# hassony2/homan

Hardware: AMD Instinct MI355X
Metric: optimisation iters/sec (30-frame 256^2 clip) (higher is better)
Workload: dtype f32

## Files before the change

### homan_amd/csrc/raster_api.hip

```cpp
#include "raster_ws.h"

RasterTune& hm_raster_tune()
{
    static thread_local RasterTune t = {0, 0, SWEEP_BLOCKS};
    return t;
}
int& hm_sweep_cap_override()
{
    static int cap = 0;
    return cap;
}
static hipEvent_t g_tev[6];
static int g_timing = 0;
#define HM_TIME_MARK(k, stream) do { if (g_timing) (void)hipEventRecord(g_tev[k], stream); } while (0)

extern "C" {

size_t hm_sil_workspace_bytes(int B, int V, int F, int S)
{
    const size_t is = 2 * (size_t)S;
    size_t n = 256;
    n += al256((size_t)B * 16);
    n += al256((size_t)B * V * 3 * 4);
    n += al256((size_t)B * F * 9 * 4);
    n += al256((size_t)B * F * 8);
    n += al256((size_t)B * is * is * 4);
    n += al256((size_t)B * is * (is / 16) * 2);
    n += al256((size_t)B * S * S * 4);
    n += al256((size_t)B * (S / 8) * (S / 8) * 16);
    n += al256((size_t)B * is * is * 4);
    n += al256((size_t)B * is * (is / 16) * 4);
    n += al256((size_t)B * is * (is / 16) * 4);
    n += al256((size_t)B * F * 24 * 4);
    n += al256((size_t)B * F * 2);
    n += al256((size_t)B * SR_MAX * 8);
    n += al256((size_t)B * (S / 16) * (S / 16));
    n += al256((size_t)B * SR_MAX * F * 4);
    n += al256(4 * (size_t)B * is * (is / 64) * 16);
    n += al256((size_t)B * 2 * is * 16);
    n += al256(4 * (size_t)B * is * is * sizeof(SweepSrc));
    n += al256((size_t)B * F * sizeof(SweepFace));
    n += al256((size_t)B * F * 4) * 2;
    n += al256(sweep_ucap(B, F) * 4);
    n += al256(sweep_slot_cap(B, F) * 24);
    n += al256(ts_units(B, F, S) * 16);
    n += al256(ts_raster_units(B, S) * 4) * 3;
    return n;
}

int hm_tune_raster_lds_pad(int bytes)
{
    const int prev = hm_raster_tune().raster_lds_pad;
    if (bytes >= 0) hm_raster_tune().raster_lds_pad = bytes;
    return prev;
}
int hm_tune_raster_reorder(int enable)
{
    const int prev = hm_raster_tune().raster_reorder;
    if (enable >= 0) hm_raster_tune().raster_reorder = enable ? 1 : 0;
    return prev;
}

int hm_tune_sweep_blocks(int blocks)
{
    const int prev = hm_raster_tune().sweep_blocks;
    if (blocks > 0) hm_raster_tune().sweep_blocks = blocks;
    return prev;
}

int hm_sil_fwd_phase_clips(const float* verts, const int* faces, int faces_bstride, const float* K, int B, int V, int F, int S,
                           float orig_size, float znear, float zfar, const float* keep, const float* ref,
                           const float* keep_sum, float* pooled, float* loss_out, const int* work_order, float* pooled_depth,
                           float* alpha_full, int mask_shared, const float* rigid_rot6d, const float* rigid_trans,
                           const float* rigid_scale, int rigid_abs, int persistent_outputs, void* workspace, int clip_len,
                           int out_stride, float* cam_verts_out, int phases, hipStream_t stream)
{
    HM_CHECK_ARG(phases >= 1 && phases <= 3);
    HM_CHECK_ARG(verts && faces && K && pooled && workspace && HM_CLIP_LEN_OK(B, clip_len));
    if (clip_len == 0) clip_len = B;
// ... 318 lines not shown
```

### homan_amd/csrc/raster_lines.hip

```cpp
#include "raster_ws.h"

__global__ __launch_bounds__(256) void k_bwd_masks(const float* __restrict__ gin, int mode,
                                                   const float* __restrict__ upstream,
                                                   const float* __restrict__ keep_sum, int B, int S,
                                                   const unsigned short* __restrict__ alpha16,
                                                   float* __restrict__ gimg, unsigned short* __restrict__ planes,
                                                   int clip_len)
{
    if (mode == 1 && upstream[0] > 0.0f) return;
    const int w = threadIdx.x >> 6, lane = threadIdx.x & 63;
    const int is = 2 * S, tiles_x = S / HM_TILE, ntiles = tiles_x * tiles_x;
    const int tile = blockIdx.x * 4 + w, b = blockIdx.y;
    if (tile >= ntiles) return;
    const int ty = tile / tiles_x, tx = tile % tiles_x;
    const int rr = lane >> 3, cc = lane & 7;
    const int r = ty * HM_TILE + rr, c = tx * HM_TILE + cc;
    const long po = ((long)b * S + r) * S + c;
    unsigned long long cq[4];
#pragma unroll
    for (int dy = 0; dy < 2; ++dy) {
        const unsigned aw = alpha16[(((long)b * (is / 16) + ty) * (is / 16) + tx) * 16 + 2 * rr + dy];
#pragma unroll
        for (int dx = 0; dx < 2; ++dx) cq[2 * dy + dx] = __ballot((aw >> (2 * cc + dx)) & 1u);
    }
// ... 75 lines not shown
    __shared__ unsigned long long s_base;
    const int tid = threadIdx.x, lane = tid & 63, wv = tid >> 6;
    const int per_clip = nblk / (B / clip_len), clip = blk / per_clip;
    const long cbase = (long)clip * clip_len * F;
    const long bf0 = cbase + ((long)(blk - clip * per_clip) * 256 + tid) * fpt, nbf = cbase + (long)clip_len * F;
    int nk[4], n = 0, hasf = 0;
#pragma unroll
    for (int k = 0; k < 4; ++k) {
        SweepFace rec;
        nk[k] = (k < fpt && bf0 + k < nbf) ? sweep_face_record(bf0 + k, faces9, boxes, owned, F, is, rec) : 0;
        n += nk[k];
        hasf += nk[k] > 0 ? 1 : 0;
    }
    const int inc_i = hm_wave_scan_incl(n), inc_f = hm_wave_scan_incl(hasf);
    if (lane == 63) { s_wsum[wv][0] = inc_i; s_wsum[wv][1] = inc_f; }
    __syncthreads();
    int pre_i = 0, pre_f = 0, tot_i = 0, tot_f = 0;
#pragma unroll
    for (int k = 0; k < 4; ++k) {
        if (k < wv) { pre_i += s_wsum[k][0]; pre_f += s_wsum[k][1]; }
        tot_i += s_wsum[k][0];
        tot_f += s_wsum[k][1];
    }
    if (tid == 0)
        s_base = tot_f ? atomicAdd(sl.cnt, ((unsigned long long)tot_f << 32) | (unsigned)((tot_i + SWEEP_UNIT - 1) & ~(SWEEP_UNIT - 1))) : 0ull;
    __syncthreads();
    const unsigned long long base = s_base;
    int off = (int)(base & 0xffffffffull) + pre_i + inc_i - n;
    int idx = (int)(base >> 32) + pre_f + inc_f - hasf;
#pragma unroll
    for (int k = 0; k < 4; ++k) {
        const long bf = bf0 + k;
        if (k >= fpt || bf >= nbf) break;
        bool zero = nk[k] == 0;
        if (nk[k] > 0) {
            SweepFace rec;
            const int nn = sweep_face_record(bf, faces9, boxes, owned, F, is, rec);
            const int u_lo = off >> SWEEP_USHIFT, u_hi = (off + nn - 1) >> SWEEP_USHIFT;
            const bool over = u_hi >= sl.ucap || u_hi + idx >= sl.slot_cap;
            rec.off = off;
            rec.flags = over ? 1 : 0;
            zero = u_hi > u_lo;
            const uint4* r4 = reinterpret_cast<const uint4*>(&rec);
            uint4* t4 = reinterpret_cast<uint4*>(sl.tab + idx);
#pragma unroll
            for (int q = 0; q < 4; ++q) t4[q] = r4[q];
            sl.offs[idx] = off;
            for (int u = (off + SWEEP_UNIT - 1) >> SWEEP_USHIFT; (u << SWEEP_USHIFT) < off + nn && u < sl.ucap; ++u)
                sl.ufirst[u] = (unsigned)idx;
            off += nn;
            ++idx;
        }
        if (zero) {
            double* o = parts + bf * 6;
#pragma unroll
            for (int q = 0; q < 6; ++q) o[q] = 0.0;
        }
    }
    if (tid == 0) {
        const unsigned int t = atomicAdd(sl.done, 1u);
        if (t == (unsigned)nblk - 1u) {
            sl.total[0] = atomicExch(sl.cnt, 0ull);
            atomicExch(sl.done, 0u);
        }
    }
}


#ifndef LINES_NL
#define LINES_NL 2
#endif
#ifdef LINES_REVERSED
#define LINES_BLK(i, n) ((n) - 1 - (i))
#else
#define LINES_BLK(i, n) (i)
#endif
template <bool W32>
__global__ __launch_bounds__(256) void k_bwd_lines(const unsigned short* __restrict__ planes,
                                                   const float* __restrict__ gimg, const float* __restrict__ dimg,
                                                   int mode, const float* __restrict__ upstream,
                                                   const float* __restrict__ keep_sum,
                                                   const int* __restrict__ idx_map, int B, int S,
                                                   SweepSrc* __restrict__ srcs, uint4* __restrict__ lrec,
                                                   int ncomp, int fpt, const float* __restrict__ faces9,
                                                   const FaceBox* __restrict__ boxes,
                                                   const unsigned char* __restrict__ owned, int F,
// ... 165 lines not shown
```

### homan_amd/csrc/raster_sweep.hip

```cpp
#include "raster_ws.h"
#include "raster_hooks.h"

__device__ __forceinline__ float sample_grad(const float* __restrict__ gimg, int S, int is, int xi, int yi)
{
    return 0.25f * gimg[(long)((is - 1 - yi) >> 1) * S + (xi >> 1)];
}

__device__ __forceinline__ void sweep_term(float diff, int d1, float d1_cross, float k0, float k1, bool use0, bool use1,
                                           float eps, double magic, double& acc0, double& acc1)
{
    const float t = (float)d1 - d1_cross;
    const bool live = diff > 0.0f;
    float dist0 = k0 * t, dist1 = k1 * t;
    dist0 += (0.0f < dist0) ? eps : -eps;
    dist1 += (0.0f < dist1) ? eps : -eps;
    const float g0 = diff / dist0, g1 = diff / dist1;
    acc0 -= hm_quant((live && use0) ? g0 : 0.0f, magic);
    acc1 -= hm_quant((live && use1) ? g1 : 0.0f, magic);
}
__device__ __forceinline__ float sweep_item_scale(float c, float two_over_is, bool pow2, int is)
{
    return pow2 ? (c * 2.0f) * two_over_is : (c * 2.0f) / (float)is;
}

__device__ __forceinline__ void raster_reorder(int* __restrict__ wo_dyn, int* __restrict__ wo_tmp,
                                               const unsigned int* __restrict__ wg_cost, unsigned int* __restrict__ dyn_flag, int n,
                                               unsigned* __restrict__ s_hist)
{
    __shared__ unsigned s_wsum[4];
    __shared__ unsigned s_zero;
    const int tid = threadIdx.x, lane = tid & 63, wv = tid >> 6;
    for (int i = tid; i < 1024; i += 256) s_hist[i] = 0u;
    if (tid == 0) s_zero = 0u;
    __syncthreads();
// ... 125 lines not shown
    q.geo = geo;
    return q;
}

#ifndef SWEEP_COMBINE_MIN
#define SWEEP_COMBINE_MIN 32
#endif
#ifndef SWEEP_COMBINE_PAIRS
#define SWEEP_COMBINE_PAIRS 192
#endif
__device__ __forceinline__ double sweep_row_sum(double v)
{
    v += hm_dpp_f64<0xb1, 0xf>(v);
    v += hm_dpp_f64<0x4e, 0xf>(v);
    v += hm_dpp_f64<0x114, 0xf>(v);
    v += hm_dpp_f64<0x118, 0xf>(v);
    return v;
}
__device__ __forceinline__ void sweep_combine_rows(int& cur, double& acc0, double& acc1, bool flush, int lane)
{
    const unsigned long long nb = __ballot(flush);
    if (__popcll(nb) < SWEEP_COMBINE_MIN) return;
    const int prev = __builtin_amdgcn_update_dpp(cur, cur, 0x111, 0xf, 0xf, false);
    const unsigned long long same = __ballot(prev == cur);
    const int sh = lane & 48;
    const bool uni = ((unsigned)(nb >> sh) & (unsigned)(same >> sh) & 0xffffu) == 0xffffu;
    const double r0 = sweep_row_sum(acc0), r1 = sweep_row_sum(acc1);
    if (uni) {
        if ((lane & 15) == 15) { acc0 = r0; acc1 = r1; }
        else { cur = -1; acc0 = 0.0; acc1 = 0.0; }
    }
}

#ifndef SWEEP_WAVES_EU
#define SWEEP_WAVES_EU 5
#endif
template <bool W32>
__global__ __launch_bounds__(256) __attribute__((amdgpu_waves_per_eu(SWEEP_WAVES_EU, 8))) void k_bwd_sweep(SweepList sl, const int* __restrict__ idx_map,
                                                   const SweepSrc* __restrict__ srcs,
                                                   const uint4* __restrict__ lrec, int B, int F, int S,
                                                   float eps, double magic, double* __restrict__ parts,
                                                   const unsigned short* __restrict__ lsum,
                                                   const unsigned short* __restrict__ alpha16,
                                                   const unsigned int* __restrict__ ts_flag,
                                                   unsigned long long* __restrict__ ts_slots, int nsort,
                                                   int* __restrict__ wo_dyn, int* __restrict__ wo_tmp,
                                                   const unsigned int* __restrict__ wg_cost,
                                                   unsigned int* __restrict__ dyn_flag, int n_wo)
{
    HM_CHAIN_KERNEL();
    typedef typename HmOff<W32>::t OFF;
    const unsigned long long ts_t0 = (unsigned long long)wall_clock64();
    const bool ts_on = hm_ts_enabled(ts_flag) && (threadIdx.x & 63) == 0;
    if (ts_on) hm_ts_store(ts_slots, (long)blockIdx.x * 4 + (threadIdx.x >> 6), 0, ts_t0);
    struct FaceLds { SweepFace f; int pad; };
    struct ItemLds { SweepItem it; int pad; };
    __shared__ FaceLds s_face[4][SWEEP_PASS_FACES];
    __shared__ double s_fg[4][SWEEP_PASS_FACES][6];
    __shared__ int s_start[4][64];
    __shared__ int s_head[4][256];
    __shared__ ItemLds s_item[4][64];
    __shared__ unsigned short s_q[4][SWEEP_UNIT];
    __shared__ int2 s_fam[4][SWEEP_PASS_FACES][12];
    __shared__ int s_fb[4][SWEEP_PASS_FACES][2];
    if (nsort && blockIdx.x == 0) {
        raster_reorder(wo_dyn, wo_tmp, wg_cost, dyn_flag, n_wo, reinterpret_cast<unsigned*>(&s_head[0][0]));
        if (ts_on) hm_ts_store(ts_slots, (long)blockIdx.x * 4 + (threadIdx.x >> 6), 1, (unsigned long long)wall_clock64());
        return;
    }
    const int wid = (int)blockIdx.x - nsort, nwork = (int)gridDim.x - nsort;
    const int lane = threadIdx.x & 63, wv = threadIdx.x >> 6;
    const int is = 2 * S;
    const bool pow2 = (is & (is - 1)) == 0;
    const float inv_is = 1.0f / (float)is;
    const int wpl = is / 64;
    const unsigned long long tot = sl.total[0];
    const int N = (int)(tot & 0xffffffffull), W = (int)(tot >> 32);
    const int U = (N + SWEEP_UNIT - 1) >> SWEEP_USHIFT;
    const int xcd = wid & 7;
    const int xwaves = (nwork >> 3) * 4;
    const int u_end = (int)(((long)U * (xcd + 1)) >> 3);
    int first_ahead = -1;
    for (int u = __builtin_amdgcn_readfirstlane((int)(((long)U * xcd) >> 3) + (wid >> 3) * 4 + wv); u < u_end;
         u += xwaves) {
        const int ubeg = u << SWEEP_USHIFT, uend = ubeg + SWEEP_UNIT;
#ifdef SWEEP_UNIT_PROFILE
        const unsigned long long up_t0 = wall_clock64();
        int up_pass = 0, up_trips = 0, up_q = 0, up_rounds = 0;
#endif
        int first = first_ahead;
        if (first < 0) {
            if (u < sl.ucap) first = (int)sl.ufirst[u];
            else {
                int lo = 0, hi = W - 1;
                while (lo < hi) {
                    const int mid = (lo + hi + 1) >> 1;
                    if (sl.offs[mid] <= ubeg) lo = mid; else hi = mid - 1;
                }
                first = lo;
            }
            first = __builtin_amdgcn_readfirstlane(first);
        }
        const int u_ahead = u + xwaves;
        int ahead_v = -1;
        if (u_ahead < u_end && u_ahead < sl.ucap) ahead_v = (int)sl.ufirst[u_ahead];
        for (int fb = 0;; fb += SWEEP_PASS_FACES) {
            const int o = (lane <= SWEEP_PASS_FACES && first + fb + lane < W) ? sl.offs[first + fb + lane] : 0x7fffffff;
            int row[SWEEP_PASS_FACES / 4];
#pragma unroll
            for (int k = 0; k < SWEEP_PASS_FACES / 4; ++k) {
                const int fi = first + fb + 4 * k + (lane >> 4);
                row[k] = fi < W ? reinterpret_cast<const int*>(sl.tab + fi)[lane & 15] : 0;
            }
            if (fb == 0) first_ahead = __builtin_amdgcn_readfirstlane(ahead_v);
            const int nfp = __popcll(__ballot(lane < SWEEP_PASS_FACES && o < uend));
            if (nfp == 0) break;
#ifdef SWEEP_UNIT_PROFILE
            ++up_pass;
// ... 153 lines not shown
                if (on[ph]) {
                    rf[ph] = *hm_at<W32>(lrec, lid[ph] * wpl + (rfrom[ph] >> 6));
                    rt[ph] = *hm_at<W32>(lrec, lid[ph] * wpl + (rto[ph] >> 6));
                }
            }
#pragma unroll
            for (int ph = 0; ph < 2; ++ph) {
                const unsigned long long wf = rf[ph].x | ((unsigned long long)rf[ph].y << 32);
                const unsigned long long wt = rt[ph].x | ((unsigned long long)rt[ph].y << 32);
                lo[ph] = (int)rf[ph].z + __popcll(wf & ((1ull << (rfrom[ph] & 63)) - 1ull));
                nbp[ph] = on[ph] ? (int)rt[ph].z + __popcll(wt & (~0ull >> (63 - (rto[ph] & 63)))) - lo[ph] : 0;
            }
            const int nb0 = nbp[0], nb1 = nbp[1];
#ifdef SWEEP_STATS
            {
                const unsigned long long c[7] = {__popcll(__ballot(mine)), __popcll(__ballot(geo)), __popcll(__ballot(act0)),
                                                 __popcll(__ballot(act1)), __popcll(__ballot(nb0 > 0)), __popcll(__ballot(nb1 > 0)),
                                                 (unsigned long long)hm_wave_scan_incl(nb0 + nb1)};
                if (lane == 63) { for (int k = 0; k < 7; ++k) atomicAdd(&g_sweep_n[k], c[k]); atomicAdd(&g_sweep_n[7], 1ull); }
            }
#endif
            const int n = nb0 + nb1;
            const int incl = hm_wave_scan_incl(n);
            const int npairs = __builtin_amdgcn_readlane(incl, 63);
            if (npairs > 0) {
                __builtin_amdgcn_wave_barrier();
                s_start[wv][lane] = incl - n;
                SweepItem it;
                it.x = d1_cross;
                it.c0 = sweep_item_scale(c0, inv_is, pow2, is);
                it.c1 = sweep_item_scale(c1, inv_is, pow2, is);
                it.base0 = (int)(lid[0] * is) + lo[0];
                it.base1 = (int)(lid[1] * is) + lo[1];
                it.nb0 = nb0;
                it.fn = fn;
                {
                    const int m0 = var ? 2 - edge : edge, k1 = edge == 2 ? 0 : edge + 1, m1 = var ? 2 - k1 : k1;
                    const int comp = axis ? 0 : 1;
                    it.meta = el | ((2 * m0 + comp) << 4) | ((2 * m1 + comp) << 7) | (use0 ? 1 << 10 : 0) |
                              (use1 ? 1 << 11 : 0) | (nb0 << 12);
                }
                s_item[wv][lane].it = it;
                wave_sync();
                const int* st = s_start[wv];
                int cur = -1;
                double acc0 = 0.0, acc1 = 0.0;
                int carry = 0;
#pragma unroll 1
                for (int base = 0; base < npairs; base += 256) {
                    SWEEP_HOOK_PAIR_ROUND(eps, base);
#ifdef SWEEP_STATS
                    if (lane == 0) atomicAdd(&g_sweep_n[11], 1ull);
#endif
#ifdef SWEEP_UNIT_PROFILE
                    ++up_rounds;
#endif
                    int4* hd = reinterpret_cast<int4*>(s_head[wv]);
                    hd[lane] = make_int4(0, 0, 0, 0);
                    wave_sync();
                    const int ex = incl - n;
                    if (n > 0 && ex >= base && ex < base + 256) s_head[wv][ex - base] = lane + 1;
                    wave_sync();
                    const int4 h = hd[lane];
                    int m[4];
                    m[0] = h.x; m[1] = max(m[0], h.y); m[2] = max(m[1], h.z); m[3] = max(m[2], h.w);
                    int inc = m[3];
                    inc = max(inc, __builtin_amdgcn_update_dpp(0, inc, 0x111, 0xf, 0xf, false));
                    inc = max(inc, __builtin_amdgcn_update_dpp(0, inc, 0x112, 0xf, 0xf, false));
                    inc = max(inc, __builtin_amdgcn_update_dpp(0, inc, 0x114, 0xf, 0xf, false));
                    inc = max(inc, __builtin_amdgcn_update_dpp(0, inc, 0x118, 0xf, 0xf, false));
                    inc = max(inc, __builtin_amdgcn_update_dpp(0, inc, 0x142, 0xa, 0xf, false));
                    inc = max(inc, __builtin_amdgcn_update_dpp(0, inc, 0x143, 0xc, 0xf, false));
                    int before = __builtin_amdgcn_update_dpp(0, inc, 0x138, 0xf, 0xf, false);
                    before = max(before, carry);
                    carry = max(carry, __builtin_amdgcn_readlane(inc, 63));
                    SweepSrc sc[4];
                    int qi[4], qmeta[4];
                    bool ph1[4];
#pragma unroll
                    for (int k = 0; k < 4; ++k) {
                        const int p = min(base + 4 * lane + k, npairs - 1);
                        const int i = max(max(before, m[k]) - 1, 0);
                        const int r = max(p - st[i], 0);
                        const SweepItem& qq = s_item[wv][i].it;
                        qmeta[k] = qq.meta;
                        const int q_nb0 = qmeta[k] >> 12;
                        ph1[k] = r >= q_nb0;
                        qi[k] = i;
                        OFF at = (OFF)qq.base0 + r;
                        if (ph1[k]) at = (OFF)qq.base1 + (r - q_nb0);
                        sc[k] = *hm_at<W32>(srcs, at);
                    }
#if SWEEP_COMBINE_MIN <= 64
                    if (base > 0) {
                        const int key0 = base + 4 * lane < npairs ? (qmeta[0] & 0x3ff) : cur;
                        sweep_combine_rows(cur, acc0, acc1, cur >= 0 && key0 != cur, lane);
                    }
#endif
#pragma unroll
                    for (int k = 0; k < 4; ++k) {
                        {
                            const bool valid = base + 4 * lane + k < npairs;
                            const SweepItem& qq = s_item[wv][qi[k]].it;
                            const int meta = qmeta[k], key = valid ? (meta & 0x3ff) : cur;
                            if (key != cur) {
                                if (cur >= 0) {
#ifdef SWEEP_HOOK_FLUSH
                                    SWEEP_HOOK_FLUSH(eps, s_fg[wv], lane, cur, acc0, acc1);
#else
                                    double* f = s_fg[wv][cur & 15];
                                    unsafeAtomicAdd(f + ((cur >> 4) & 7), acc0);
                                    unsafeAtomicAdd(f + ((cur >> 7) & 7), acc1);
#endif
                                }
                                cur = key;
                                acc0 = 0.0;
                                acc1 = 0.0;
                            }
                            const bool take = valid && (!ph1[k] || sc[k].owner == qq.fn);
                            sweep_term(take ? (ph1[k] ? sc[k].g : -sc[k].g) : 0.0f, sc[k].d1, qq.x, qq.c0, qq.c1,
                                       (meta & (1 << 10)) != 0, (meta & (1 << 11)) != 0, eps, magic, acc0, acc1);
                        }
                    }
                }
#if SWEEP_COMBINE_MIN <= 64
                if (npairs >= SWEEP_COMBINE_PAIRS) sweep_combine_rows(cur, acc0, acc1, cur >= 0, lane);
#endif
                if (cur >= 0) {
                    double* f = s_fg[wv][cur & 15];
                    unsafeAtomicAdd(f + ((cur >> 4) & 7), acc0);
                    unsafeAtomicAdd(f + ((cur >> 7) & 7), acc1);
                }
            }
            wave_sync();
            }
            if (lane < nfp) {
                const SweepFace& ff = s_face[wv][lane].f;
                const int off = ff.off, nit = (int)ff.cum[11];
                const int u_lo = off >> SWEEP_USHIFT, u_hi = (off + nit - 1) >> SWEEP_USHIFT;
                double v[6];
#pragma unroll
                for (int k = 0; k < 6; ++k) v[k] = s_fg[wv][lane][k];
                double* out = parts + (long)ff.bf * 6;
                if (u_lo == u_hi) {
#pragma unroll
                    for (int k = 0; k < 6; ++k) out[k] = v[k];
                } else {
#pragma unroll
                    for (int k = 0; k < 6; ++k) unsafeAtomicAdd(out + k, v[k]);
                }
            }
            if (nfp < SWEEP_PASS_FACES) break;
        }
#ifdef SWEEP_UNIT_PROFILE
        if (lane == 0 && u < 65536) {
            g_unit_prof[u][0] = (int)(wall_clock64() - up_t0); g_unit_prof[u][1] = up_pass;
            g_unit_prof[u][2] = up_trips | (up_q << 8); g_unit_prof[u][3] = up_rounds;
        }
#endif
    }
    if (ts_on) hm_ts_store(ts_slots, (long)blockIdx.x * 4 + (threadIdx.x >> 6), 1, (unsigned long long)wall_clock64());
}

__global__ void k_bwd_gather(const double* __restrict__ parts, const int* __restrict__ adj_off,
                             const int* __restrict__ adj_items, const float* __restrict__ verts,
                             const float* __restrict__ K, int B, int V, int F, float orig_size,
                             float* __restrict__ grad_ndc, float* __restrict__ grad_verts)
{
    const long i = (long)blockIdx.x * blockDim.x + threadIdx.x;
    if (i >= (long)B * V) return;
    const int b = (int)(i / V), v = (int)(i % V);
    double su = 0.0, sv = 0.0;
    const double2* pf = reinterpret_cast<const double2*>(parts + (long)b * F * 6);
    const int a1 = adj_off[v + 1];
    for (int a = adj_off[v]; a < a1; a += 8) {
        int item[8];
#pragma unroll
        for (int k = 0; k < 8; ++k) item[k] = a + k < a1 ? adj_items[a + k] : -1;
        double2 g2[8];
#pragma unroll
        for (int k = 0; k < 8; ++k) g2[k] = item[k] >= 0 ? pf[item[k]] : make_double2(0.0, 0.0);
#pragma unroll
        for (int k = 0; k < 8; ++k) { su += g2[k].x; sv += g2[k].y; }
    }
    const float gu = (float)su, gv = (float)sv;
    if (grad_ndc) { grad_ndc[3 * i] = gu; grad_ndc[3 * i + 1] = gv; grad_ndc[3 * i + 2] = 0.f; }
    const float* k = K + b * 9;
    const float x = verts[3 * i], y = verts[3 * i + 1], z = verts[3 * i + 2];
    const float zz = z + 1e-9f;
    const float du0 = gu * (2.0f / orig_size), dv0 = -gv * (2.0f / orig_size);
    const float dxn = k[0] * du0 + k[3] * dv0;
    const float dyn = k[1] * du0 + k[4] * dv0;
    grad_verts[3 * i] = dxn / zz;
    grad_verts[3 * i + 1] = dyn / zz;
    grad_verts[3 * i + 2] = -(dxn * x + dyn * y) / (zz * zz);
}

void hm_launch_sweep(const SilWs& w, int B, int F, int S, float eps, int sum_log2q, hipStream_t stream)
{
    const RasterTune& tune = hm_raster_tune();
    const int nsort = tune.raster_reorder ? 1 : 0;
    const int blocks = max(8, (min(min(hm_cdiv((long)B * F, 2), tune.sweep_blocks), TS_SWEEP_WGS - 8) & ~7) - 8 * nsort);
    const bool w32 = hm_offsets_fit_32(B, S);
    hipLaunchKernelGGL(w32 ? k_bwd_sweep<true> : k_bwd_sweep<false>, dim3(nsort + blocks), dim3(256), 0, stream, w.sweep,
                       w.idx_map, w.srcs, w.lrec, B, F, S, eps, hm_sum_magic(sum_log2q), w.parts, w.lsum, w.alpha16, w.counter + 24,
                       w.ts + 2 * (ts_raster_units(B, S) + ts_lines_units(B, F, S)), nsort, w.wo_dyn, w.wo_tmp, w.wg_cost,
                       w.counter + 26, (int)ts_raster_units(B, S));
}
void hm_launch_bwd_gather(const SilWs& w, const int* adj_off, const int* adj_items, const float* verts, const float* K, int B,
                          int V, int F, float orig_size, float* grad_ndc, float* grad_verts, hipStream_t stream)
{
    hipLaunchKernelGGL(k_bwd_gather, dim3(hm_cdiv((long)B * V, 256)), dim3(256), 0, stream, w.parts, adj_off, adj_items, verts,
                       K, B, V, F, orig_size, grad_ndc, grad_verts);
}
int hm_sweep_occupancy(int* blocks_per_cu)
{
    return hipOccupancyMaxActiveBlocksPerMultiprocessor(blocks_per_cu, k_bwd_sweep<true>, 256, 0) == hipSuccess ? HM_OK : HM_ERR_LAUNCH;
}
#ifdef SWEEP_UNIT_PROFILE
extern "C" int hm_debug_unit_profile(int* out)
{
    (void)hipDeviceSynchronize();
    (void)hipMemcpyFromSymbol(out, HIP_SYMBOL(g_unit_prof), sizeof(int) * 65536 * 4);
    static int z[65536][4];
    (void)hipMemcpyToSymbol(HIP_SYMBOL(g_unit_prof), z, sizeof(z));
    return HM_OK;
}
#endif
#ifdef SWEEP_STATS
extern "C" int hm_debug_sweep_stats(unsigned long long* out)
{
    unsigned long long z[16] = {0, 0, 0, 0, 0, 0, 0, 0, 0, 0, 0, 0, 0, 0, 0, 0};
    (void)hipDeviceSynchronize();
    (void)hipMemcpyFromSymbol(out, HIP_SYMBOL(g_sweep_n), sizeof(z));
    (void)hipMemcpyToSymbol(HIP_SYMBOL(g_sweep_n), z, sizeof(z));
    return HM_OK;
}
#endif
```

### homan_amd/csrc/raster_ws.h

```cpp
#pragma once
#include "raster_common.h"

#define HM_INTERNAL __attribute__((visibility("hidden")))

#ifndef SWEEP_BLOCKS
#define SWEEP_BLOCKS 1280
#endif
struct RasterTune {
    int raster_lds_pad;
    int raster_reorder;
    int sweep_blocks;
};
HM_INTERNAL RasterTune& hm_raster_tune();
HM_INTERNAL int& hm_sweep_cap_override();
#define TS_SWEEP_WGS 4096
static inline size_t ts_raster_units(int B, int S) { return (size_t)B * (S / 8) * (S / 8) / RASTER_WAVES; }
static inline size_t ts_lines_units(int B, int F, int S) { return (size_t)B * F / 256 + 2 * (size_t)B + 64 + (size_t)B * S / 2 + 8; }
static inline size_t ts_units(int B, int F, int S) { return ts_raster_units(B, S) + ts_lines_units(B, F, S) + 4 * TS_SWEEP_WGS; }
static inline size_t sweep_ucap(int B, int F) { return (size_t)B * F * 4 + 1024; }
static inline size_t sweep_slot_cap(int B, int F) { return sweep_ucap(B, F) + (size_t)B * F; }

static inline size_t al256(size_t x) { return (x + 255) & ~(size_t)255; }

struct SilWs {
    unsigned int* counter; float* frame_rec;
    float* ndc; float* faces9; FaceBox* boxes; int* idx_map; unsigned short* alpha16; float* dimg;
    float* partials; float* gimg; unsigned short* planes; double* parts;
    unsigned char* owned; int* bin_cnt; unsigned int* bin_done; unsigned char* region_state; int* bin_list;
    uint4* lrec; SweepSrc* srcs; unsigned short* lsum;
    SweepList sweep;
    unsigned long long* ts;
    int* wo_dyn; int* wo_tmp; unsigned int* wg_cost;
};
static inline SilWs carve(void* ws, int B, int V, int F, int S)
{
    const size_t is = 2 * (size_t)S;
    char* p = (char*)ws;
    SilWs w;
    w.counter = (unsigned int*)p; p += 256;
    w.frame_rec = (float*)p; p += al256((size_t)B * 16);
    w.ndc = (float*)p; p += al256((size_t)B * V * 3 * 4);
    w.faces9 = (float*)p; p += al256((size_t)B * F * 9 * 4);
    w.boxes = (FaceBox*)p; p += al256((size_t)B * F * 8);
    w.idx_map = (int*)p; p += al256((size_t)B * is * is * 4);
    w.alpha16 = (unsigned short*)p; p += al256((size_t)B * is * (is / 16) * 2);
    w.dimg = (float*)p; p += al256((size_t)B * S * S * 4);
    w.partials = (float*)p; p += al256((size_t)B * (S / 8) * (S / 8) * 16);
    w.gimg = (float*)p; p += al256((size_t)B * is * is * 4);
    w.planes = (unsigned short*)p; p += al256((size_t)B * is * (is / 16) * 4) * 2;
    w.parts = (double*)p; p += al256((size_t)B * F * 24 * 4);
    w.owned = (unsigned char*)p; p += al256((size_t)B * F * 2);
    w.bin_cnt = (int*)p; w.bin_done = (unsigned int*)(p + (size_t)B * SR_MAX * 4); p += al256((size_t)B * SR_MAX * 8);
    w.region_state = (unsigned char*)p; p += al256((size_t)B * (S / 16) * (S / 16));
    w.bin_list = (int*)p; p += al256((size_t)B * SR_MAX * F * 4);
    w.lrec = (uint4*)p; p += al256(4 * (size_t)B * is * (is / 64) * 16);
    w.lsum = (unsigned short*)p; p += al256((size_t)B * 2 * is * 16);
    w.srcs = (SweepSrc*)p; p += al256(4 * (size_t)B * is * is * sizeof(SweepSrc));
    w.sweep.tab = (SweepFace*)p; p += al256((size_t)B * F * sizeof(SweepFace));
    w.sweep.offs = (int*)p; p += al256((size_t)B * F * 4);
    w.sweep.tickets = (unsigned int*)p; p += al256((size_t)B * F * 4);
    w.sweep.ufirst = (unsigned int*)p; p += al256(sweep_ucap(B, F) * 4);
    w.sweep.upart = (float*)p; p += al256(sweep_slot_cap(B, F) * 24);
    w.ts = (unsigned long long*)p; p += al256(ts_units(B, F, S) * 16);
    w.wo_dyn = (int*)p; p += al256(ts_raster_units(B, S) * 4);
    w.wo_tmp = (int*)p; p += al256(ts_raster_units(B, S) * 4);
    w.wg_cost = (unsigned int*)p;
    w.sweep.cnt = (unsigned long long*)(w.counter + 16);
    w.sweep.done = w.counter + 18;
    w.sweep.total = (unsigned long long*)(w.counter + 20);
    w.sweep.ucap = (int)sweep_ucap(B, F);
    w.sweep.slot_cap = (int)sweep_slot_cap(B, F);
    if (hm_sweep_cap_override() > 0) {
        w.sweep.ucap = min(w.sweep.ucap, hm_sweep_cap_override());
        w.sweep.slot_cap = min(w.sweep.slot_cap, hm_sweep_cap_override());
    }
    return w;
}

static inline bool hm_offsets_fit_32(int B, int S)
{
    static const bool force64 = [] { const char* e = getenv("HOMAN_FORCE_W64"); return e && atoi(e) != 0; }();
    return !force64 && 4.0 * B * (2.0 * S) * (2.0 * S) * sizeof(SweepSrc) < 4.0e9;
}

HM_INTERNAL void hm_launch_setup_faces(const SilWs& w, const float* verts, const float* K, float orig_size, const int* faces,
                                       int faces_bstride, int B, int V, int F, int is, int* bins, const float* rigid_rot6d,
                                       const float* rigid_trans, const float* rigid_scale, int rigid_abs, int clip_len,
                                       float* cam_verts_out, hipStream_t stream);
#define HM_MAX_RENDERS 4
struct SetupFacesArgs {
    const float* verts; const float* K; float orig_size; const int* faces; int faces_bstride; int B, V, F, is; int* bins;
    const float* rigid_rot6d; const float* rigid_trans; const float* rigid_scale; int rigid_abs; int clip_len; float* cam_verts_out;
};
struct SetupFacesK {
    const float* verts; const float* K; float orig_size; const int* faces; int faces_bstride; int B, V, F, is; float* faces9;
    FaceBox* boxes; unsigned char* owned; int* bin_cnt; int* bin_list; const float* rigid_rot6d; const float* rigid_trans;
    const float* rigid_scale; int rigid_abs; int clip_len; float* cam_out; int nfb;
};
struct SetupFacesMulti { SetupFacesK r[HM_MAX_RENDERS]; int first[HM_MAX_RENDERS + 1]; int nblk[HM_MAX_RENDERS]; int n; };
HM_INTERNAL void hm_launch_setup_faces_multi(const SilWs* w, const SetupFacesArgs* a, int n, hipStream_t stream);
struct RasterFwdArgs {
    int B, F, S;
    float znear, zfar;
    float* pooled; const float* keep; const float* ref; bool fused;
    const int* work_order; float* pooled_depth; int* bins; int reset_bins; int persistent; float* alpha_full; int mask_shared;
// ... 29 lines not shown
```

Baseline: 6610.

## Split backward sweep into item emission and pair-balanced walk kernel

The sweep kernel now writes surviving edge items for units below a capacity to a global buffer, together with per-unit and per-slice pair counts, instead of processing pairs inline. A new walk kernel uses a prefix sum over those counts to give each workgroup an equal range of pairs, clipping items at the range edges, and accumulates face gradients via atomics. The goal is to fix load imbalance caused by a few heavy units. It costs an extra launch, global traffic for the item buffer, and unconditional zeroing of per-face partials in the lines kernel.

```diff
diff --git a/homan_amd/csrc/raster_api.hip b/homan_amd/csrc/raster_api.hip
--- a/homan_amd/csrc/raster_api.hip
+++ b/homan_amd/csrc/raster_api.hip
@@ -45,6 +45,10 @@
     n += al256(sweep_slot_cap(B, F) * 24);
     n += al256(ts_units(B, F, S) * 16);
     n += al256(ts_raster_units(B, S) * 4) * 3;
+    n += al256(sweep_scap(B, S) * SWEEP_UNIT * sizeof(SweepItem));
+    n += al256(sweep_scap(B, S) * SWEEP_UNIT * 4);
+    n += al256(sweep_scap(B, S) * 8);
+    n += al256((size_t)TS_SWEEP_WGS * 8);
     return n;
 }
 
diff --git a/homan_amd/csrc/raster_lines.hip b/homan_amd/csrc/raster_lines.hip
--- a/homan_amd/csrc/raster_lines.hip
+++ b/homan_amd/csrc/raster_lines.hip
@@ -131,15 +131,13 @@
     for (int k = 0; k < 4; ++k) {
         const long bf = bf0 + k;
         if (k >= fpt || bf >= nbf) break;
-        bool zero = nk[k] == 0;
         if (nk[k] > 0) {
             SweepFace rec;
             const int nn = sweep_face_record(bf, faces9, boxes, owned, F, is, rec);
-            const int u_lo = off >> SWEEP_USHIFT, u_hi = (off + nn - 1) >> SWEEP_USHIFT;
+            const int u_hi = (off + nn - 1) >> SWEEP_USHIFT;
             const bool over = u_hi >= sl.ucap || u_hi + idx >= sl.slot_cap;
             rec.off = off;
             rec.flags = over ? 1 : 0;
-            zero = u_hi > u_lo;
             const uint4* r4 = reinterpret_cast<const uint4*>(&rec);
             uint4* t4 = reinterpret_cast<uint4*>(sl.tab + idx);
 #pragma unroll
@@ -150,7 +148,7 @@
             off += nn;
             ++idx;
         }
-        if (zero) {
+        {
             double* o = parts + bf * 6;
 #pragma unroll
             for (int q = 0; q < 6; ++q) o[q] = 0.0;
diff --git a/homan_amd/csrc/raster_sweep.hip b/homan_amd/csrc/raster_sweep.hip
--- a/homan_amd/csrc/raster_sweep.hip
+++ b/homan_amd/csrc/raster_sweep.hip
@@ -1,5 +1,6 @@
 #include "raster_ws.h"
 #include "raster_hooks.h"
+#include "sweep_split.h"
 
 __device__ __forceinline__ float sample_grad(const float* __restrict__ gimg, int S, int is, int xi, int yi)
 {
@@ -191,6 +192,104 @@
     }
 }
 
+struct SweepItemLds { SweepItem it; int pad; };
+template <bool W32>
+__device__ __forceinline__ void sweep_pair_rounds(const int* st, int* head, const SweepItemLds* items, double (*fg)[6],
+                                                  const SweepSrc* __restrict__ srcs, int lane, int incl, int n, int npairs,
+                                                  float eps, double magic, int& rounds)
+{
+    typedef typename HmOff<W32>::t OFF;
+    (void)rounds;
+    int cur = -1;
+    double acc0 = 0.0, acc1 = 0.0;
+    int carry = 0;
+#pragma unroll 1
+    for (int base = 0; base < npairs; base += 256) {
+        SWEEP_HOOK_PAIR_ROUND(eps, base);
+#ifdef SWEEP_STATS
+        if (lane == 0) atomicAdd(&g_sweep_n[11], 1ull);
+#endif
+#ifdef SWEEP_UNIT_PROFILE
+        ++rounds;
+#endif
+        int4* hd = reinterpret_cast<int4*>(head);
+        hd[lane] = make_int4(0, 0, 0, 0);
+        wave_sync();
+        const int ex = incl - n;
+        if (n > 0 && ex >= base && ex < base + 256) head[ex - base] = lane + 1;
+        wave_sync();
+        const int4 h = hd[lane];
+        int m[4];
+        m[0] = h.x; m[1] = max(m[0], h.y); m[2] = max(m[1], h.z); m[3] = max(m[2], h.w);
+        int inc = m[3];
+        inc = max(inc, __builtin_amdgcn_update_dpp(0, inc, 0x111, 0xf, 0xf, false));
+        inc = max(inc, __builtin_amdgcn_update_dpp(0, inc, 0x112, 0xf, 0xf, false));
+        inc = max(inc, __builtin_amdgcn_update_dpp(0, inc, 0x114, 0xf, 0xf, false));
+        inc = max(inc, __builtin_amdgcn_update_dpp(0, inc, 0x118, 0xf, 0xf, false));
+        inc = max(inc, __builtin_amdgcn_update_dpp(0, inc, 0x142, 0xa, 0xf, false));
+        inc = max(inc, __builtin_amdgcn_update_dpp(0, inc, 0x143, 0xc, 0xf, false));
+        int before = __builtin_amdgcn_update_dpp(0, inc, 0x138, 0xf, 0xf, false);
+        before = max(before, carry);
+        carry = max(carry, __builtin_amdgcn_readlane(inc, 63));
+        SweepSrc sc[4];
+        int qi[4], qmeta[4];
+        bool ph1[4];
+#pragma unroll
+        for (int k = 0; k < 4; ++k) {
+            const int p = min(base + 4 * lane + k, npairs - 1);
+            const int i = max(max(before, m[k]) - 1, 0);
+            const int r = max(p - st[i], 0);
+            const SweepItem& qq = items[i].it;
+            qmeta[k] = qq.meta;
+            const int q_nb0 = qmeta[k] >> 12;
+            ph1[k] = r >= q_nb0;
+            qi[k] = i;
+            OFF at = (OFF)qq.base0 + r;
+            if (ph1[k]) at = (OFF)qq.base1 + (r - q_nb0);
+            sc[k] = *hm_at<W32>(srcs, at);
+        }
+#if SWEEP_COMBINE_MIN <= 64
+        if (base > 0) {
+            const int key0 = base + 4 * lane < npairs ? (qmeta[0] & 0x3ff) : cur;
+            sweep_combine_rows(cur, acc0, acc1, cur >= 0 && key0 != cur, lane);
+        }
+#endif
+#pragma unroll
+        for (int k = 0; k < 4; ++k) {
+            {
+                const bool valid = base + 4 * lane + k < npairs;
+                const SweepItem& qq = items[qi[k]].it;
+                const int meta = qmeta[k], key = valid ? (meta & 0x3ff) : cur;
+                if (key != cur) {
+                    if (cur >= 0) {
+#ifdef SWEEP_HOOK_FLUSH
+                        SWEEP_HOOK_FLUSH(eps, fg, lane, cur, acc0, acc1);
+#else
+                        double* f = fg[cur & 15];
+                        unsafeAtomicAdd(f + ((cur >> 4) & 7), acc0);
+                        unsafeAtomicAdd(f + ((cur >> 7) & 7), acc1);
+#endif
+                    }
+                    cur = key;
+                    acc0 = 0.0;
+                    acc1 = 0.0;
+                }
+                const bool take = valid && (!ph1[k] || sc[k].owner == qq.fn);
+                sweep_term(take ? (ph1[k] ? sc[k].g : -sc[k].g) : 0.0f, sc[k].d1, qq.x, qq.c0, qq.c1,
+                           (meta & (1 << 10)) != 0, (meta & (1 << 11)) != 0, eps, magic, acc0, acc1);
+            }
+        }
+    }
+#if SWEEP_COMBINE_MIN <= 64
+    if (npairs >= SWEEP_COMBINE_PAIRS) sweep_combine_rows(cur, acc0, acc1, cur >= 0, lane);
+#endif
+    if (cur >= 0) {
+        double* f = fg[cur & 15];
+        unsafeAtomicAdd(f + ((cur >> 4) & 7), acc0);
+        unsafeAtomicAdd(f + ((cur >> 7) & 7), acc1);
+    }
+}
+
 #ifndef SWEEP_WAVES_EU
 #define SWEEP_WAVES_EU 5
 #endif
@@ -205,7 +304,9 @@
                                                    unsigned long long* __restrict__ ts_slots, int nsort,
                                                    int* __restrict__ wo_dyn, int* __restrict__ wo_tmp,
                                                    const unsigned int* __restrict__ wg_cost,
-                                                   unsigned int* __restrict__ dyn_flag, int n_wo)
+                                                   unsigned int* __restrict__ dyn_flag, int n_wo,
+                                                   SweepItem* __restrict__ surv, int* __restrict__ surv_bf,
+                                                   int2* __restrict__ utab, unsigned long long* __restrict__ gtab, int scap)
 {
     HM_CHAIN_KERNEL();
     typedef typename HmOff<W32>::t OFF;
@@ -213,7 +314,7 @@
     const bool ts_on = hm_ts_enabled(ts_flag) && (threadIdx.x & 63) == 0;
     if (ts_on) hm_ts_store(ts_slots, (long)blockIdx.x * 4 + (threadIdx.x >> 6), 0, ts_t0);
     struct FaceLds { SweepFace f; int pad; };
-    struct ItemLds { SweepItem it; int pad; };
+    typedef SweepItemLds ItemLds;
     __shared__ FaceLds s_face[4][SWEEP_PASS_FACES];
     __shared__ double s_fg[4][SWEEP_PASS_FACES][6];
     __shared__ int s_start[4][64];
@@ -222,6 +323,7 @@
     __shared__ unsigned short s_q[4][SWEEP_UNIT];
     __shared__ int2 s_fam[4][SWEEP_PASS_FACES][12];
     __shared__ int s_fb[4][SWEEP_PASS_FACES][2];
+    __shared__ unsigned long long s_wpairs[4];
     if (nsort && blockIdx.x == 0) {
         raster_reorder(wo_dyn, wo_tmp, wg_cost, dyn_flag, n_wo, reinterpret_cast<unsigned*>(&s_head[0][0]));
         if (ts_on) hm_ts_store(ts_slots, (long)blockIdx.x * 4 + (threadIdx.x >> 6), 1, (unsigned long long)wall_clock64());
@@ -236,13 +338,15 @@
     const unsigned long long tot = sl.total[0];
     const int N = (int)(tot & 0xffffffffull), W = (int)(tot >> 32);
     const int U = (N + SWEEP_UNIT - 1) >> SWEEP_USHIFT;
-    const int xcd = wid & 7;
-    const int xwaves = (nwork >> 3) * 4;
-    const int u_end = (int)(((long)U * (xcd + 1)) >> 3);
+    const int slice = (wid & 7) * (nwork >> 3) + (wid >> 3);
+    const int xwaves = 4;
+    const int u_end = hm_split_slice_begin(U, slice + 1, nwork);
+    unsigned long long wave_pairs = 0ull;
     int first_ahead = -1;
-    for (int u = __builtin_amdgcn_readfirstlane((int)(((long)U * xcd) >> 3) + (wid >> 3) * 4 + wv); u < u_end;
-         u += xwaves) {
+    for (int u = __builtin_amdgcn_readfirstlane(hm_split_slice_begin(U, slice, nwork) + wv); u < u_end; u += xwaves) {
         const int ubeg = u << SWEEP_USHIFT, uend = ubeg + SWEEP_UNIT;
+        const bool handover = u < scap;
+        int u_surv = 0, u_pairs = 0;
 #ifdef SWEEP_UNIT_PROFILE
         const unsigned long long up_t0 = wall_clock64();
         int up_pass = 0, up_trips = 0, up_q = 0, up_rounds = 0;
@@ -462,7 +566,7 @@
                 it.c1 = sweep_item_scale(c1, inv_is, pow2, is);
                 it.base0 = (int)(lid[0] * is) + lo[0];
                 it.base1 = (int)(lid[1] * is) + lo[1];
-                it.nb0 = nb0;
+                it.nb0 = handover ? n : nb0;
                 it.fn = fn;
                 {
                     const int m0 = var ? 2 - edge : edge, k1 = edge == 2 ? 0 : edge + 1, m1 = var ? 2 - k1 : k1;
@@ -470,101 +574,29 @@
                     it.meta = el | ((2 * m0 + comp) << 4) | ((2 * m1 + comp) << 7) | (use0 ? 1 << 10 : 0) |
                               (use1 ? 1 << 11 : 0) | (nb0 << 12);
                 }
+                if (handover) {
+                    const unsigned long long kb = __ballot(n > 0);
+                    if (n > 0) {
+                        const long at = (long)ubeg + u_surv + __popcll(kb & ((1ull << lane) - 1ull));
+                        uint4* dst = reinterpret_cast<uint4*>(surv + at);
+                        dst[0] = make_uint4(__float_as_uint(it.x), __float_as_uint(it.c0), __float_as_uint(it.c1), (unsigned)it.base0);
+                        dst[1] = make_uint4((unsigned)it.base1, (unsigned)it.nb0, (unsigned)it.fn, (unsigned)it.meta);
+                        surv_bf[at] = fc.bf;
+                    }
+                    u_surv += __popcll(kb);
+                    u_pairs += npairs;
+                } else {
                 s_item[wv][lane].it = it;
                 wave_sync();
-                const int* st = s_start[wv];
-                int cur = -1;
-                double acc0 = 0.0, acc1 = 0.0;
-                int carry = 0;
-#pragma unroll 1
-                for (int base = 0; base < npairs; base += 256) {
-                    SWEEP_HOOK_PAIR_ROUND(eps, base);
-#ifdef SWEEP_STATS
-                    if (lane == 0) atomicAdd(&g_sweep_n[11], 1ull);
-#endif
-#ifdef SWEEP_UNIT_PROFILE
-                    ++up_rounds;
-#endif
-                    int4* hd = reinterpret_cast<int4*>(s_head[wv]);
-                    hd[lane] = make_int4(0, 0, 0, 0);
-                    wave_sync();
-                    const int ex = incl - n;
-                    if (n > 0 && ex >= base && ex < base + 256) s_head[wv][ex - base] = lane + 1;
-                    wave_sync();
-                    const int4 h = hd[lane];
-                    int m[4];
-                    m[0] = h.x; m[1] = max(m[0], h.y); m[2] = max(m[1], h.z); m[3] = max(m[2], h.w);
-                    int inc = m[3];
-                    inc = max(inc, __builtin_amdgcn_update_dpp(0, inc, 0x111, 0xf, 0xf, false));
-                    inc = max(inc, __builtin_amdgcn_update_dpp(0, inc, 0x112, 0xf, 0xf, false));
-                    inc = max(inc, __builtin_amdgcn_update_dpp(0, inc, 0x114, 0xf, 0xf, false));
-                    inc = max(inc, __builtin_amdgcn_update_dpp(0, inc, 0x118, 0xf, 0xf, false));
-                    inc = max(inc, __builtin_amdgcn_update_dpp(0, inc, 0x142, 0xa, 0xf, false));
-                    inc = max(inc, __builtin_amdgcn_update_dpp(0, inc, 0x143, 0xc, 0xf, false));
-                    int before = __builtin_amdgcn_update_dpp(0, inc, 0x138, 0xf, 0xf, false);
-                    before = max(before, carry);
-                    carry = max(carry, __builtin_amdgcn_readlane(inc, 63));
-                    SweepSrc sc[4];
-                    int qi[4], qmeta[4];
-                    bool ph1[4];
-#pragma unroll
-                    for (int k = 0; k < 4; ++k) {
-                        const int p = min(base + 4 * lane + k, npairs - 1);
-                        const int i = max(max(before, m[k]) - 1, 0);
-                        const int r = max(p - st[i], 0);
-                        const SweepItem& qq = s_item[wv][i].it;
-                        qmeta[k] = qq.meta;
-                        const int q_nb0 = qmeta[k] >> 12;
-                        ph1[k] = r >= q_nb0;
-                        qi[k] = i;
-                        OFF at = (OFF)qq.base0 + r;
-                        if (ph1[k]) at = (OFF)qq.base1 + (r - q_nb0);
-                        sc[k] = *hm_at<W32>(srcs, at);
-                    }
-#if SWEEP_COMBINE_MIN <= 64
-                    if (base > 0) {
-                        const int key0 = base + 4 * lane < npairs ? (qmeta[0] & 0x3ff) : cur;
-                        sweep_combine_rows(cur, acc0, acc1, cur >= 0 && key0 != cur, lane);
-                    }
-#endif
-#pragma unroll
-                    for (int k = 0; k < 4; ++k) {
-                        {
-                            const bool valid = base + 4 * lane + k < npairs;
-                            const SweepItem& qq = s_item[wv][qi[k]].it;
-                            const int meta = qmeta[k], key = valid ? (meta & 0x3ff) : cur;
-                            if (key != cur) {
-                                if (cur >= 0) {
-#ifdef SWEEP_HOOK_FLUSH
-                                    SWEEP_HOOK_FLUSH(eps, s_fg[wv], lane, cur, acc0, acc1);
-#else
-                                    double* f = s_fg[wv][cur & 15];
-                                    unsafeAtomicAdd(f + ((cur >> 4) & 7), acc0);
-                                    unsafeAtomicAdd(f + ((cur >> 7) & 7), acc1);
-#endif
-                                }
-                                cur = key;
-                                acc0 = 0.0;
-                                acc1 = 0.0;
-                            }
-                            const bool take = valid && (!ph1[k] || sc[k].owner == qq.fn);
-                            sweep_term(take ? (ph1[k] ? sc[k].g : -sc[k].g) : 0.0f, sc[k].d1, qq.x, qq.c0, qq.c1,
-                                       (meta & (1 << 10)) != 0, (meta & (1 << 11)) != 0, eps, magic, acc0, acc1);
-                        }
-                    }
-                }
-#if SWEEP_COMBINE_MIN <= 64
-                if (npairs >= SWEEP_COMBINE_PAIRS) sweep_combine_rows(cur, acc0, acc1, cur >= 0, lane);
-#endif
-                if (cur >= 0) {
-                    double* f = s_fg[wv][cur & 15];
-                    unsafeAtomicAdd(f + ((cur >> 4) & 7), acc0);
-                    unsafeAtomicAdd(f + ((cur >> 7) & 7), acc1);
+#ifndef SWEEP_UNIT_PROFILE
+                int up_rounds = 0;
+#endif
+                sweep_pair_rounds<W32>(s_start[wv], s_head[wv], s_item[wv], s_fg[wv], srcs, lane, incl, n, npairs, eps, magic, up_rounds);
                 }
             }
             wave_sync();
             }
-            if (lane < nfp) {
+            if (!handover && lane < nfp) {
                 const SweepFace& ff = s_face[wv][lane].f;
                 const int off = ff.off, nit = (int)ff.cum[11];
                 const int u_lo = off >> SWEEP_USHIFT, u_hi = (off + nit - 1) >> SWEEP_USHIFT;
@@ -582,6 +614,10 @@
             }
             if (nfp < SWEEP_PASS_FACES) break;
         }
+        if (handover) {
+            if (lane == 0) utab[u] = make_int2(u_surv, u_pairs);
+            wave_pairs += (unsigned long long)u_pairs;
+        }
 #ifdef SWEEP_UNIT_PROFILE
         if (lane == 0 && u < 65536) {
             g_unit_prof[u][0] = (int)(wall_clock64() - up_t0); g_unit_prof[u][1] = up_pass;
@@ -589,7 +625,140 @@
         }
 #endif
     }
-    if (ts_on) hm_ts_store(ts_slots, (long)blockIdx.x * 4 + (threadIdx.x >> 6), 1, (unsigned long long)wall_clock64());
+    if (lane == 0) s_wpairs[wv] = wave_pairs;
+    __syncthreads();
+    if (threadIdx.x == 0) gtab[slice] = s_wpairs[0] + s_wpairs[1] + s_wpairs[2] + s_wpairs[3];
+}
+
+template <bool W32>
+__global__ __launch_bounds__(256) void k_bwd_sweep_walk(const unsigned long long* __restrict__ total,
+                                                        const SweepItem* __restrict__ surv, const int* __restrict__ surv_bf,
+                                                        const int2* __restrict__ utab,
+                                                        const unsigned long long* __restrict__ gtab, int nslices, int scap,
+                                                        const SweepSrc* __restrict__ srcs, float eps, double magic,
+                                                        double* __restrict__ parts, const unsigned int* __restrict__ ts_flag,
+                                                        unsigned long long* __restrict__ ts_slots, int ts_first)
+{
+    HM_CHAIN_KERNEL();
+    const bool ts_on = hm_ts_enabled(ts_flag) && (threadIdx.x & 63) == 0;
+    __shared__ double s_fg[4][SWEEP_PASS_FACES][6];
+    __shared__ int s_start[4][64];
+    __shared__ int s_head[4][256];
+    __shared__ SweepItemLds s_item[4][64];
+    __shared__ int s_bf[4][SWEEP_PASS_FACES];
+    __shared__ unsigned long long s_pre[256];
+    __shared__ unsigned long long s_wsum[4];
+    const int tid = threadIdx.x, lane = tid & 63, wv = tid >> 6;
+    const int N = (int)(total[0] & 0xffffffffull);
+    const int Uall = (N + SWEEP_UNIT - 1) >> SWEEP_USHIFT, U = min(Uall, scap);
+    const int per = (nslices + 255) >> 8;
+    unsigned long long mysum = 0ull;
+    for (int k = 0; k < per; ++k) { const int i = tid * per + k; if (i < nslices) mysum += gtab[i]; }
+    unsigned long long inc = mysum;
+#pragma unroll
+    for (int d = 1; d < 64; d <<= 1) {
+        const unsigned lo = (unsigned)__shfl_up((int)(unsigned)(inc & 0xffffffffull), d, 64);
+        const unsigned hi = (unsigned)__shfl_up((int)(unsigned)(inc >> 32), d, 64);
+        if (lane >= d) inc += ((unsigned long long)hi << 32) | lo;
+    }
+    if (lane == 63) s_wsum[wv] = inc;
+    __syncthreads();
+    unsigned long long wbase = 0ull, P = 0ull;
+#pragma unroll
+    for (int k = 0; k < 4; ++k) { if (k < wv) wbase += s_wsum[k]; P += s_wsum[k]; }
+    s_pre[tid] = wbase + inc - mysum;
+    __syncthreads();
+    const int nwork = (int)gridDim.x;
+    const int wpos = ((int)blockIdx.x & 7) * (nwork >> 3) + ((int)blockIdx.x >> 3);
+    const unsigned long long p0 = hm_split_bound(P, wpos * 4 + wv, nwork * 4), p1 = hm_split_bound(P, wpos * 4 + wv + 1, nwork * 4);
+    if (p0 < p1) {
+        int cnt = 0;
+#pragma unroll
+        for (int k = 0; k < 4; ++k) cnt += __popcll(__ballot(hm_split_starts_before(s_pre[64 * k + lane], p0)));
+        const int chunk = cnt - 1;
+        unsigned long long sv = 0ull;
+        if (lane < per && chunk * per + lane < nslices) sv = gtab[chunk * per + lane];
+        unsigned long long sinc = sv;
+#pragma unroll
+        for (int d = 1; d < 16; d <<= 1) {
+            const unsigned lo = (unsigned)__shfl_up((int)(unsigned)(sinc & 0xffffffffull), d, 64);
+            const unsigned hi = (unsigned)__shfl_up((int)(unsigned)(sinc >> 32), d, 64);
+            if (lane >= d) sinc += ((unsigned long long)hi << 32) | lo;
+        }
+        const unsigned long long sex = s_pre[chunk] + sinc - sv;
+        const int scnt = __popcll(__ballot(lane < per && chunk * per + lane < nslices && hm_split_starts_before(sex, p0)));
+        const int slice = chunk * per + scnt - 1;
+        unsigned long long pos = ((unsigned long long)(unsigned)__builtin_amdgcn_readlane((int)(unsigned)(sex >> 32), scnt - 1) << 32) |
+                                 (unsigned)__builtin_amdgcn_readlane((int)(unsigned)(sex & 0xffffffffull), scnt - 1);
+        bool done = false;
+        for (int ub = hm_split_slice_begin(Uall, slice, nslices); ub < U && !done; ub += 64) {
+            const int2 ue = ub + lane < U ? utab[ub + lane] : make_int2(0, 0);
+            const int uinc = hm_wave_scan_incl(ue.y);
+            const unsigned long long ufirst = pos + (unsigned long long)(uinc - ue.y);
+            unsigned long long todo = __ballot(ue.y > 0 && ufirst + (unsigned long long)ue.y > p0 && ufirst < p1);
+            while (todo) {
+                const int j = __builtin_amdgcn_readfirstlane(__builtin_ctzll(todo));
+                todo &= todo - 1ull;
+                const int u = ub + j, nsurv = __builtin_amdgcn_readlane(ue.x, j);
+                unsigned long long e = pos + (unsigned long long)(unsigned)__builtin_amdgcn_readlane(uinc - ue.y, j);
+                for (int k = 0; k < nsurv;) {
+                    const bool have = k + lane < nsurv;
+                    const long at = ((long)u << SWEEP_USHIFT) + k + lane;
+                    uint4 r0 = make_uint4(0u, 0u, 0u, 0u), r1 = r0;
+                    int bf = -1;
+                    if (have) {
+                        const uint4* src = reinterpret_cast<const uint4*>(surv + at);
+                        r0 = src[0];
+                        r1 = src[1];
+                        bf = surv_bf[at];
+                    }
+                    const int bf_prev = __builtin_amdgcn_update_dpp(bf, bf, 0x138, 0xf, 0xf, false);
+                    const unsigned long long hb = __ballot(have && (lane == 0 || bf != bf_prev));
+                    const int el = __popcll(hb & (~0ull >> (63 - lane))) - 1;
+                    const bool ok = have && el < SWEEP_PASS_FACES;
+                    const unsigned long long okb = __ballot(ok);
+                    const int len = __popcll(okb);
+                    const int nfaces = __popcll(hb & okb);
+                    const int nfull = ok ? (int)r1.y : 0, meta0 = (int)r1.w;
+                    const int finc = hm_wave_scan_incl(nfull);
+                    const HmSplitClip c = hm_split_clip(e + (unsigned long long)(finc - nfull), nfull, meta0 >> 12, p0, p1);
+                    e += (unsigned long long)(unsigned)__builtin_amdgcn_readlane(finc, 63);
+                    k += len;
+                    const int n = c.m0 + c.m1;
+                    const int incl = hm_wave_scan_incl(n);
+                    const int npairs = __builtin_amdgcn_readlane(incl, 63);
+                    if (npairs > 0) {
+                        __builtin_amdgcn_wave_barrier();
+                        s_start[wv][lane] = incl - n;
+                        SweepItem it;
+                        it.x = __uint_as_float(r0.x); it.c0 = __uint_as_float(r0.y); it.c1 = __uint_as_float(r0.z);
+                        it.base0 = (int)r0.w + c.a0;
+                        it.base1 = (int)r1.x + c.a1;
+                        it.nb0 = c.m0;
+                        it.fn = (int)r1.z;
+                        it.meta = (meta0 & 0xff0) | (el & 15) | (c.m0 << 12);
+                        s_item[wv][lane].it = it;
+                        for (int i = lane; i < SWEEP_PASS_FACES * 6; i += 64) (&s_fg[wv][0][0])[i] = 0.0;
+                        if (ok && ((hb >> lane) & 1ull)) s_bf[wv][el] = bf;
+                        wave_sync();
+                        int rounds = 0;
+                        sweep_pair_rounds<W32>(s_start[wv], s_head[wv], s_item[wv], s_fg[wv], srcs, lane, incl, n, npairs, eps, magic, rounds);
+                        wave_sync();
+                        for (int i = lane; i < nfaces * 6; i += 64) {
+                            const int f = i / 6, q = i - 6 * f;
+                            const double v = s_fg[wv][f][q];
+                            if (v != 0.0) unsafeAtomicAdd(parts + (long)s_bf[wv][f] * 6 + q, v);
+                        }
+                        wave_sync();
+                    }
+                    if (e >= p1) break;
+                }
+            }
+            pos += (unsigned long long)(unsigned)__builtin_amdgcn_readlane(uinc, 63);
+            done = pos >= p1;
+        }
+    }
+    if (ts_on) hm_ts_store(ts_slots, (long)(ts_first + (int)blockIdx.x) * 4 + (threadIdx.x >> 6), 1, (unsigned long long)wall_clock64());
 }
 
 __global__ void k_bwd_gather(const double* __restrict__ parts, const int* __restrict__ adj_off,
@@ -632,10 +801,14 @@
     const int nsort = tune.raster_reorder ? 1 : 0;
     const int blocks = max(8, (min(min(hm_cdiv((long)B * F, 2), tune.sweep_blocks), TS_SWEEP_WGS - 8) & ~7) - 8 * nsort);
     const bool w32 = hm_offsets_fit_32(B, S);
+    unsigned long long* ts_slots = w.ts + 2 * (ts_raster_units(B, S) + ts_lines_units(B, F, S));
     hipLaunchKernelGGL(w32 ? k_bwd_sweep<true> : k_bwd_sweep<false>, dim3(nsort + blocks), dim3(256), 0, stream, w.sweep,
                        w.idx_map, w.srcs, w.lrec, B, F, S, eps, hm_sum_magic(sum_log2q), w.parts, w.lsum, w.alpha16, w.counter + 24,
-                       w.ts + 2 * (ts_raster_units(B, S) + ts_lines_units(B, F, S)), nsort, w.wo_dyn, w.wo_tmp, w.wg_cost,
-                       w.counter + 26, (int)ts_raster_units(B, S));
+                       ts_slots, nsort, w.wo_dyn, w.wo_tmp, w.wg_cost, w.counter + 26, (int)ts_raster_units(B, S), w.surv,
+                       w.surv_bf, w.utab, w.gtab, w.scap);
+    hipLaunchKernelGGL(w32 ? k_bwd_sweep_walk<true> : k_bwd_sweep_walk<false>, dim3(blocks), dim3(256), 0, stream,
+                       (const unsigned long long*)w.sweep.total, w.surv, w.surv_bf, w.utab, w.gtab, blocks, w.scap, w.srcs, eps,
+                       hm_sum_magic(sum_log2q), w.parts, w.counter + 24, ts_slots, nsort);
 }
 void hm_launch_bwd_gather(const SilWs& w, const int* adj_off, const int* adj_items, const float* verts, const float* K, int B,
                           int V, int F, float orig_size, float* grad_ndc, float* grad_verts, hipStream_t stream)
diff --git a/homan_amd/csrc/raster_ws.h b/homan_amd/csrc/raster_ws.h
--- a/homan_amd/csrc/raster_ws.h
+++ b/homan_amd/csrc/raster_ws.h
@@ -19,6 +19,7 @@
 static inline size_t ts_units(int B, int F, int S) { return ts_raster_units(B, S) + ts_lines_units(B, F, S) + 4 * TS_SWEEP_WGS; }
 static inline size_t sweep_ucap(int B, int F) { return (size_t)B * F * 4 + 1024; }
 static inline size_t sweep_slot_cap(int B, int F) { return sweep_ucap(B, F) + (size_t)B * F; }
+static inline size_t sweep_scap(int B, int S) { return (size_t)B * 2 * S + 64; }
 
 static inline size_t al256(size_t x) { return (x + 255) & ~(size_t)255; }
 
@@ -31,6 +32,7 @@
     SweepList sweep;
     unsigned long long* ts;
     int* wo_dyn; int* wo_tmp; unsigned int* wg_cost;
+    SweepItem* surv; int* surv_bf; int2* utab; unsigned long long* gtab; int scap;
 };
 static inline SilWs carve(void* ws, int B, int V, int F, int S)
 {
@@ -64,13 +66,19 @@
     w.ts = (unsigned long long*)p; p += al256(ts_units(B, F, S) * 16);
     w.wo_dyn = (int*)p; p += al256(ts_raster_units(B, S) * 4);
     w.wo_tmp = (int*)p; p += al256(ts_raster_units(B, S) * 4);
-    w.wg_cost = (unsigned int*)p;
+    w.wg_cost = (unsigned int*)p; p += al256(ts_raster_units(B, S) * 4);
+    w.scap = (int)sweep_scap(B, S);
+    w.surv = (SweepItem*)p; p += al256((size_t)w.scap * SWEEP_UNIT * sizeof(SweepItem));
+    w.surv_bf = (int*)p; p += al256((size_t)w.scap * SWEEP_UNIT * 4);
+    w.utab = (int2*)p; p += al256((size_t)w.scap * 8);
+    w.gtab = (unsigned long long*)p;
     w.sweep.cnt = (unsigned long long*)(w.counter + 16);
     w.sweep.done = w.counter + 18;
     w.sweep.total = (unsigned long long*)(w.counter + 20);
     w.sweep.ucap = (int)sweep_ucap(B, F);
     w.sweep.slot_cap = (int)sweep_slot_cap(B, F);
     if (hm_sweep_cap_override() > 0) {
+        w.scap = min(w.scap, hm_sweep_cap_override());
         w.sweep.ucap = min(w.sweep.ucap, hm_sweep_cap_override());
         w.sweep.slot_cap = min(w.sweep.slot_cap, hm_sweep_cap_override());
     }
diff --git a/homan_amd/csrc/sweep_split.h b/homan_amd/csrc/sweep_split.h
--- /dev/null
+++ b/homan_amd/csrc/sweep_split.h
@@ -0,0 +1,53 @@
+#pragma once
+#if defined(__HIPCC__) || defined(__CUDACC__)
+#define HM_SPLIT_HD __host__ __device__ __forceinline__
+#else
+#define HM_SPLIT_HD static inline
+#endif
+
+HM_SPLIT_HD int hm_split_slice_begin(int U, int s, int ns) { return (int)(((long long)U * s) / ns); }
+
+HM_SPLIT_HD unsigned long long hm_split_bound(unsigned long long P, int w, int W) { return (P * (unsigned long long)w) / (unsigned long long)W; }
+
+HM_SPLIT_HD bool hm_split_starts_before(unsigned long long excl, unsigned long long p) { return excl <= p; }
+
+struct HmSplitClip { int a0, m0, a1, m1; };
+HM_SPLIT_HD HmSplitClip hm_split_clip(unsigned long long gp, int n, int nb0, unsigned long long p0, unsigned long long p1)
+{
+    const long long lo = (long long)p0 - (long long)gp, hi = (long long)p1 - (long long)gp;
+    const int a = (int)(lo < 0 ? 0 : (lo > n ? n : lo)), b = (int)(hi < 0 ? 0 : (hi > n ? n : hi));
+    HmSplitClip c;
+    const int s0 = a < nb0 ? a : nb0, e0 = b < nb0 ? b : nb0;
+    const int s1 = (a > nb0 ? a : nb0) - nb0, e1 = (b > nb0 ? b : nb0) - nb0;
+    c.a0 = s0; c.m0 = e0 > s0 ? e0 - s0 : 0;
+    c.a1 = s1; c.m1 = e1 > s1 ? e1 - s1 : 0;
+    return c;
+}
+
+struct HmSplitStart { int slice, unit; unsigned long long unit_first, p0, p1; };
+HM_SPLIT_HD bool hm_split_locate(const unsigned long long* slice_pairs, int ns, const int* unit_pairs, int U, int w, int W,
+                                 HmSplitStart* out)
+{
+    unsigned long long P = 0;
+    for (int s = 0; s < ns; ++s) P += slice_pairs[s];
+    out->p0 = hm_split_bound(P, w, W);
+    out->p1 = hm_split_bound(P, w + 1, W);
+    if (out->p0 >= out->p1) return false;
+    unsigned long long excl = 0, first = 0;
+    int slice = 0;
+    for (int s = 0; s < ns; ++s) {
+        if (hm_split_starts_before(excl, out->p0)) { slice = s; first = excl; }
+        excl += slice_pairs[s];
+    }
+    const int ub = hm_split_slice_begin(U, slice, ns), ue = hm_split_slice_begin(U, slice + 1, ns);
+    int unit = ub;
+    excl = first;
+    for (int u = ub; u < ue; ++u) {
+        if (hm_split_starts_before(excl, out->p0)) { unit = u; first = excl; }
+        excl += (unsigned long long)unit_pairs[u];
+    }
+    out->slice = slice;
+    out->unit = unit;
+    out->unit_first = first;
+    return true;
+}
```

New measurement: 5254. 20.5% lower.
